# jack-nie/bitcoin-miner

Hardware: AMD Instinct MI355X
Metric: GH/s (SHA-256 nonce search) at 1/2/4/8 MI355X; % of VALU int roofline (higher is better)
Workload: dtype u32

## Files before the change

### bitcoin-miner_amd/csrc/minehip.cpp

```cpp
#include <hip/hip_runtime.h>
#include <stdio.h>
#include <stdlib.h>
#include <string.h>

#include <algorithm>
#include <atomic>
#include <chrono>
#include <cmath>
#include <condition_variable>
#include <memory>
#include <mutex>
#include <string>
#include <system_error>
#include <thread>
#include <vector>

#include "../../include/minehip.h"
#include "../../include/minehip_server.h"
#include "layout.hpp"
#include "msgcodec.hpp"
#include "multi.hpp"
#include "plan.hpp"
#include "sched.hpp"

namespace mh {
hipError_t fast_module_init(int dev);
#ifdef MH_DEV_HOOKS
hipError_t fast_keep_ok(int dev, bool* ok);
#endif
hipError_t launch_fast(int dev, int J, int mode, const FastArgs& a, Partial* partials, hipStream_t s);
hipError_t launch_generic_scan(const GenArgs& a, Partial* partials, uint32_t blocks, hipStream_t s);
hipError_t launch_hash_batch(const GenArgs& a, const uint64_t* d_nonces, uint64_t* d_out, uint64_t n,
                             hipStream_t s);
hipError_t launch_merge(const Partial* partials, uint32_t n, Partial* best, hipStream_t s);
hipError_t launch_batch_scan(const BatchEntry* entries, const uint32_t* tile_entry, Partial* partials, uint32_t tiles,
                             hipStream_t s);
hipError_t launch_merge_segments(const Partial* partials, const uint32_t* seg, Partial* results, uint32_t requests,
                                 hipStream_t s);
}

namespace {

using mh::Partial;

thread_local std::string g_err;

int fail(int code, const std::string& what) {
    g_err = what;
    return code;
}

}

namespace mh {
int set_error(int code, const char* what) { return fail(code, what); }
}

namespace {

#define MH_HIP(call)                                                                                 \
    do {                                                                                             \
        hipError_t e_ = (call);                                                                      \
        if (e_ != hipSuccess) return fail(MH_EHIP, std::string(#call) + ": " + hipGetErrorString(e_)); \
    } while (0)

constexpr uint64_t kBatchChunk = 1u << 22;
constexpr int kEventPairs = 512;
constexpr uint32_t kQueueSlots = 4096;
constexpr size_t kBatchTableBytes = 4u << 20;
constexpr uint32_t kBatchResults = 1u << 16;

struct Timed {
    hipEvent_t start = nullptr, stop = nullptr;
    int kind;
    int var;
};

struct VarStat {
    uint64_t launches = 0, nonces = 0, ns = 0, ops = 0, slots = 0;
};
constexpr int kVariants = 16 * mh::kModes * 5;
inline int var_index(int J, int mode, int L) { return J + 16 * mode + 16 * mh::kModes * (L - 1); }

struct DevCtx {
    std::mutex mu;
    int dev = -1;
    bool ready = false;
    hipStream_t stream = nullptr;
    hipStream_t ps[2] = {nullptr, nullptr};
    hipEvent_t ev_piece[2] = {nullptr, nullptr};
    hipEvent_t ev_main = nullptr;
    Partial* d_partials = nullptr;
    Partial* d_best = nullptr;
    Partial* h_best = nullptr;
    uint64_t* d_nonces = nullptr;
    uint64_t* d_hashes = nullptr;
    uint32_t poff = 0;
    uint32_t* d_counters = nullptr;
    uint32_t qoff = 0;
    uint8_t* d_btab = nullptr;
    uint8_t* h_btab = nullptr;
    Partial* d_bres = nullptr;
    Partial* h_bres = nullptr;
#ifdef MH_DEV_HOOKS
    uint32_t keep = 0;
    bool keep_fast = false;
#endif
    bool prof = false;
    std::vector<Timed> pool;
    int used = 0;
    uint64_t cnt[8] = {0};
    VarStat var[kVariants];
};

std::mutex g_tab_mu;
std::vector<std::unique_ptr<DevCtx>> g_tab;
int g_ndev = -1;

int device_count_impl() {
    std::lock_guard<std::mutex> lk(g_tab_mu);
    if (g_ndev < 0) {
        int n = 0;
        if (hipGetDeviceCount(&n) != hipSuccess) n = 0;
        g_ndev = n;
        g_tab.resize((size_t)n);
        for (auto& p : g_tab) p.reset(new DevCtx());
    }
    return g_ndev;
}

int get_ctx(int dev, DevCtx** out) {
    const int n = device_count_impl();
    if (n <= 0) return fail(MH_ENODEV, "no HIP device visible");
    if (dev < 0 || dev >= n) return fail(MH_EINVAL, "device index out of range");
    DevCtx* c = g_tab[(size_t)dev].get();
    *out = c;
    return MH_OK;
}

int init_locked(DevCtx* c, int dev) {
    if (c->ready) return MH_OK;
    MH_HIP(hipSetDevice(dev));
    hipDeviceProp_t prop;
    MH_HIP(hipGetDeviceProperties(&prop, dev));
    if (strncmp(prop.gcnArchName, "gfx950", 6) != 0)
        return fail(MH_ENODEV, std::string("device is ") + prop.gcnArchName + ", kernels are built for gfx950 only");
    if (!c->stream) MH_HIP(hipStreamCreateWithFlags(&c->stream, hipStreamNonBlocking));
    if (!c->ps[0] || !c->ps[1]) {
        int least = 0, greatest = 0;
        MH_HIP(hipDeviceGetStreamPriorityRange(&least, &greatest));
        if (!c->ps[0]) MH_HIP(hipStreamCreateWithPriority(&c->ps[0], hipStreamNonBlocking, greatest));
        if (!c->ps[1]) MH_HIP(hipStreamCreateWithPriority(&c->ps[1], hipStreamNonBlocking, least));
    }
    for (auto& e : c->ev_piece)
        if (!e) MH_HIP(hipEventCreateWithFlags(&e, hipEventDisableTiming));
    if (!c->ev_main) MH_HIP(hipEventCreateWithFlags(&c->ev_main, hipEventDisableTiming));
    if (!c->d_partials) MH_HIP(hipMalloc(&c->d_partials, sizeof(Partial) * mh::kMaxBlocksPerLaunch));
    if (!c->d_best) MH_HIP(hipMalloc(&c->d_best, sizeof(Partial)));
    if (!c->d_counters) MH_HIP(hipMalloc(&c->d_counters, sizeof(uint32_t) * kQueueSlots));
    if (!c->h_best) MH_HIP(hipHostMalloc(&c->h_best, sizeof(Partial), hipHostMallocDefault));
    if (!c->d_nonces) MH_HIP(hipMalloc(&c->d_nonces, sizeof(uint64_t) * kBatchChunk));
    if (!c->d_hashes) MH_HIP(hipMalloc(&c->d_hashes, sizeof(uint64_t) * kBatchChunk));
    if (c->pool.empty()) c->pool.resize(kEventPairs);
    for (auto& t : c->pool) {
        if (!t.start) MH_HIP(hipEventCreate(&t.start));
        if (!t.stop) MH_HIP(hipEventCreate(&t.stop));
    }
    MH_HIP(mh::fast_module_init(dev));
    c->dev = dev;
    c->ready = true;
    return MH_OK;
}

#ifdef MH_DEV_HOOKS
int read_hash_keep(DevCtx* c) {
    c->keep = 0;
    c->keep_fast = false;
    const char* e = getenv("MINEHIP_DEV_HASH_KEEP");
    if (!e || !*e) return MH_OK;
    unsigned k0 = 0, k1 = 0;
    char rest = 0;
    if (sscanf(e, "%u,%u%c", &k0, &k1, &rest) != 2 || k0 > 32u || k1 > 32u)
        return fail(MH_EINVAL, "MINEHIP_DEV_HASH_KEEP: expected k0,k1 with 0 <= k <= 32");
    MH_HIP(mh::fast_keep_ok(c->dev, &c->keep_fast));
    c->keep = mh::keep_word(k0, k1);
    return MH_OK;
}
#endif

int harvest_locked(DevCtx* c) {
    for (int i = 0; i < c->used; ++i) {
        float ms = 0.f;
        MH_HIP(hipEventElapsedTime(&ms, c->pool[(size_t)i].start, c->pool[(size_t)i].stop));
        const uint64_t ns = (uint64_t)((double)ms * 1.0e6);
        c->cnt[c->pool[(size_t)i].kind == 0 ? 2 : 5] += ns;
        if (c->pool[(size_t)i].kind == 0) c->var[c->pool[(size_t)i].var].ns += ns;
    }
    c->used = 0;
    return MH_OK;
}

int piece_streams_wait_main(DevCtx* c) {
    MH_HIP(hipEventRecord(c->ev_main, c->stream));
    for (auto s : c->ps) MH_HIP(hipStreamWaitEvent(s, c->ev_main, 0));
    return MH_OK;
}

int flush_partials(DevCtx* c, bool split) {
    if (!c->poff) return MH_OK;
    if (split) {
        for (int k = 0; k < 2; ++k) {
            MH_HIP(hipEventRecord(c->ev_piece[k], c->ps[k]));
            MH_HIP(hipStreamWaitEvent(c->stream, c->ev_piece[k], 0));
        }
    }
    MH_HIP(mh::launch_merge(c->d_partials, c->poff, c->d_best, c->stream));
    c->poff = 0;
    if (split) return piece_streams_wait_main(c);
    return MH_OK;
}

bool coarse_piece(const mh::Piece& p, const mh::PlanOpts& opt) { return p.kind == 0 && p.L == opt.lower_digits; }

bool early_piece_ok(const mh::Piece& p) {
    const mh::FastArgs& a = p.fa;
    const uint32_t J = (uint32_t)p.J;
    if ((a.inner >> 2) != J || a.hole + a.hole_w > a.n_hi + a.L) return false;
    for (uint32_t j = 0; j + 1u < a.L; ++j) {
        const uint32_t pos = a.g_last - j - (j >= a.g_hole ? 1u : 0u);
        if (pos > a.g_last || (pos >> 2) != J) return false;
    }
    return true;
}

int enqueue_piece(DevCtx* c, const mh::Piece& p, const mh::PlanOpts& opt, bool split) {
    hipStream_t s = !split ? c->stream : c->ps[coarse_piece(p, opt) ? 0 : 1];
    uint32_t blocks;
    if (p.kind == 0) {
        if (p.fa.n_runs == 0 || p.fa.L < 1 || p.fa.L > 5 || p.fa.n_hi + p.fa.L > 20)
            return fail(MH_EINTERNAL, "internal: bad fast piece");
        if (p.fa.mode >= mh::kModeOneEarly && !early_piece_ok(p))
            return fail(MH_EINTERNAL, "internal: bad Early piece (an enumerated digit outside word J)");
        blocks = (p.fa.n_runs + mh::kBlockThreads - 1) / mh::kBlockThreads;
    } else {
        if (p.ga.count == 0 || p.ga.count > (uint64_t)mh::kMaxBlocksPerLaunch * mh::kBlockThreads)
            return fail(MH_EINTERNAL, "internal: bad generic piece");
        blocks = (uint32_t)((p.ga.count + mh::kBlockThreads - 1) / mh::kBlockThreads);
    }
    if (blocks > mh::kMaxBlocksPerLaunch) return fail(MH_EINTERNAL, "internal: grid too large");
    if (c->poff + blocks > mh::kMaxBlocksPerLaunch) {
        const int rc = flush_partials(c, split);
        if (rc) return rc;
    }
    Partial* out = c->d_partials + c->poff;
    Timed* tm = nullptr;
    mh::FastArgs fa = p.fa;
#ifdef MH_DEV_HOOKS
    mh::GenArgs ga = p.ga;
    ga.pad = c->keep;
    if (p.kind == 0) {
        if (c->keep && !c->keep_fast)
            return fail(MH_EINVAL, "MINEHIP_DEV_HASH_KEEP is set but the fast code object is not the coarse-hash "
                                   "variant (MINEHIP_DEV_CODE_OBJECT=build/fast_search_keep.hsaco)");
        fa.pad_ = c->keep;
    }
#else
    const mh::GenArgs& ga = p.ga;
#endif
    if (p.kind == 0) {
        fa.n_chunks = blocks;
        fa.counter = (opt.queue && c->qoff < kQueueSlots) ? c->d_counters + c->qoff++ : nullptr;
    }
    if (c->prof) {
        if (c->used == kEventPairs) {
            MH_HIP(hipStreamSynchronize(c->stream));
            for (auto ps : c->ps) MH_HIP(hipStreamSynchronize(ps));
            int rc = harvest_locked(c);
            if (rc) return rc;
        }
        tm = &c->pool[(size_t)c->used++];
        tm->kind = p.kind;
        tm->var = p.kind == 0 ? var_index(p.J, p.mode, p.L) : 0;
        MH_HIP(hipEventRecord(tm->start, s));
    }
    if (p.kind == 0)
        MH_HIP(mh::launch_fast(c->dev, p.J, p.mode, fa, out, s));
    else
        MH_HIP(mh::launch_generic_scan(ga, out, blocks, s));
    if (tm) MH_HIP(hipEventRecord(tm->stop, s));
    c->poff += blocks;
    if (c->prof) {
        if (p.kind == 0) {
            const uint64_t n = p.count;
            c->cnt[0] += 1;
            c->cnt[1] += n;
            c->cnt[3] += n * (uint64_t)p.ops;
            c->cnt[6] += n * (uint64_t)p.slots;
            VarStat& v = c->var[var_index(p.J, p.mode, p.L)];
            v.launches += 1;
            v.nonces += n;
            v.ops += n * (uint64_t)p.ops;
            v.slots += n * (uint64_t)p.slots;
        } else {
            c->cnt[4] += p.count;
        }
    }
    return MH_OK;
}

mh::PlanOpts plan_opts() {
    mh::PlanOpts o;
    if (const char* e = getenv("MINEHIP_LOWER_DIGITS")) {
        const int v = atoi(e);
        if (v >= 1 && v <= 5) o.lower_digits = v;
    }
    if (const char* e = getenv("MINEHIP_MIN_LANES")) o.min_lanes = strtoull(e, nullptr, 10);
    if (const char* e = getenv("MINEHIP_LAUNCH_NONCES")) {
        const unsigned long long v = strtoull(e, nullptr, 10);
        if (v >= 1) o.max_nonces_per_launch = v;
    }
    if (const char* e = getenv("MINEHIP_GENERIC_BELOW")) o.generic_below = strtoull(e, nullptr, 10);
    if (const char* e = getenv("MINEHIP_MAX_BLOCKS")) {
        const unsigned long long v = strtoull(e, nullptr, 10);
        if (v >= 1 && v <= mh::kMaxBlocksPerLaunch) o.max_blocks = (uint32_t)v;
    }
    if (const char* e = getenv("MINEHIP_STREAMS")) {
        const int v = atoi(e);
        if (v == 1 || v == 2) o.streams = v;
    }
    if (const char* e = getenv("MINEHIP_FINE_TAIL")) o.fine_tail = strtoull(e, nullptr, 10);
    if (const char* e = getenv("MINEHIP_QUEUE")) {
        const int v = atoi(e);
        if (v == 0 || v == 1) o.queue = v;
    }
    if (const char* e = getenv("MINEHIP_EARLY")) {
        const int v = atoi(e);
        if (v == 0 || v == 1) o.early = v;
    }
    return o;
}

uint64_t now_ns() {
    return (uint64_t)std::chrono::duration_cast<std::chrono::nanoseconds>(
               std::chrono::steady_clock::now().time_since_epoch())
        .count();
}

int search_impl(int dev, const mh::Prefix& pre, uint64_t lower, uint64_t upper, uint64_t* oh, uint64_t* on,
                uint64_t* busy_ns = nullptr) {
    DevCtx* c;
    int rc = get_ctx(dev, &c);
    if (rc) return rc;
    std::lock_guard<std::mutex> lk(c->mu);
    rc = init_locked(c, dev);
    if (rc) return rc;
    const uint64_t t0 = now_ns();
    MH_HIP(hipSetDevice(dev));
#ifdef MH_DEV_HOOKS
    rc = read_hash_keep(c);
    if (rc) return rc;
#endif
    MH_HIP(hipMemsetAsync(c->d_best, 0xFF, sizeof(Partial), c->stream));
    const mh::PlanOpts opt = plan_opts();
    if (opt.queue) MH_HIP(hipMemsetAsync(c->d_counters, 0, sizeof(uint32_t) * kQueueSlots, c->stream));
    c->qoff = 0;
    bool any_coarse = false, any_fine = false;
    if (opt.streams == 2)
        mh::plan_search(pre, lower, upper, opt, [&](const mh::Piece& p) {
            (coarse_piece(p, opt) ? any_coarse : any_fine) = true;
            return !(any_coarse && any_fine);
        });
    const bool split = opt.streams == 2 && any_coarse && any_fine;
    if (split) {
        rc = piece_streams_wait_main(c);
        if (rc) return rc;
    }
    int err = MH_OK;
    c->poff = 0;
    mh::plan_search(pre, lower, upper, opt, [&](const mh::Piece& p) {
        err = enqueue_piece(c, p, opt, split);
        return err == MH_OK;
    });
    if (!err) err = flush_partials(c, split);
    if (err) {
        for (auto ps : c->ps)
            if (ps) (void)hipStreamSynchronize(ps);
        (void)hipStreamSynchronize(c->stream);
        return err;
    }
    MH_HIP(hipMemcpyAsync(c->h_best, c->d_best, sizeof(Partial), hipMemcpyDeviceToHost, c->stream));
    MH_HIP(hipStreamSynchronize(c->stream));
    if (c->prof) {
        rc = harvest_locked(c);
        if (rc) return rc;
    }
    *oh = c->h_best->hash;
    *on = c->h_best->nonce;
    if (busy_ns) *busy_ns = now_ns() - t0;
    return MH_OK;
}

int check_common(const uint8_t* msg, size_t len) {
    if (msg == nullptr && len != 0) return fail(MH_EINVAL, "msg is NULL");
    if (len > MH_MAX_MSG_LEN) return fail(MH_ETOOLONG, "message longer than MH_MAX_MSG_LEN");
    return MH_OK;
}


uint32_t batch_slots() {
    if (const char* e = getenv("MINEHIP_BATCH_SLOTS")) {
        const unsigned long long v = strtoull(e, nullptr, 10);
        if (v >= 1 && v <= mh::kMaxBlocksPerLaunch) return (uint32_t)v;
    }
    return mh::kMaxBlocksPerLaunch;
}

inline size_t align16(size_t x) { return (x + 15u) & ~(size_t)15u; }

int batch_init_locked(DevCtx* c) {
    if (!c->d_btab) MH_HIP(hipMalloc(&c->d_btab, kBatchTableBytes));
    if (!c->h_btab) MH_HIP(hipHostMalloc(&c->h_btab, kBatchTableBytes, hipHostMallocDefault));
    if (!c->d_bres) MH_HIP(hipMalloc(&c->d_bres, sizeof(Partial) * kBatchResults));
    if (!c->h_bres) MH_HIP(hipHostMalloc(&c->h_bres, sizeof(Partial) * kBatchResults, hipHostMallocDefault));
    return MH_OK;
}

struct BatchPending {
    std::vector<size_t> req_idx;
    size_t toff = 0;
};

int batch_drain(DevCtx* c, const mh::BatchRequest* reqs, BatchPending* pend, mh_result* out) {
    MH_HIP(hipStreamSynchronize(c->stream));
    if (c->prof) {
        const int rc = harvest_locked(c);
        if (rc) return rc;
    }
    for (size_t k = 0; k < pend->req_idx.size(); ++k) {
        mh_result& r = out[reqs[pend->req_idx[k]].id];
        r.hash = c->h_bres[k].hash;
        r.nonce = c->h_bres[k].nonce;
    }
    pend->req_idx.clear();
    pend->toff = 0;
    return MH_OK;
}

int batch_run_pass(DevCtx* c, const mh::BatchRequest* reqs, const mh::BatchTables& t, uint32_t slot_cap,
                   BatchPending* pend, mh_result* out) {
    if (!mh::batch_tables_ok(t, slot_cap)) return fail(MH_EINTERNAL, "internal: bad batch tables");
    const size_t ne = t.entries.size(), nreq = t.req_idx.size(), tiles = t.tile_entry.size();
    const size_t o_seg = align16(ne * sizeof(mh::BatchEntry)), o_tile = o_seg + align16((nreq + 1u) * sizeof(uint32_t));
    const size_t bytes = o_tile + align16(tiles * sizeof(uint32_t));
    if (bytes > kBatchTableBytes || nreq > kBatchResults) return fail(MH_EINTERNAL, "internal: batch pass too large");
    if (pend->toff + bytes > kBatchTableBytes || pend->req_idx.size() + nreq > kBatchResults ||
        (c->prof && c->used == kEventPairs)) {
        const int rc = batch_drain(c, reqs, pend, out);
        if (rc) return rc;
    }
    uint8_t* h = c->h_btab + pend->toff;
    uint8_t* d = c->d_btab + pend->toff;
    memcpy(h, t.entries.data(), ne * sizeof(mh::BatchEntry));
#ifdef MH_DEV_HOOKS
    for (size_t i = 0; i < ne; ++i) ((mh::BatchEntry*)h)[i].g.pad = c->keep;
#endif
    memcpy(h + o_seg, t.seg.data(), (nreq + 1u) * sizeof(uint32_t));
    memcpy(h + o_tile, t.tile_entry.data(), tiles * sizeof(uint32_t));
    MH_HIP(hipMemcpyAsync(d, h, bytes, hipMemcpyHostToDevice, c->stream));
    Timed* tm = nullptr;
    if (c->prof) {
        tm = &c->pool[(size_t)c->used++];
        tm->kind = 1;
        tm->var = 0;
// ... 412 lines not shown
```

### bitcoin-miner_amd/csrc/plan.cpp

```cpp
#include "plan.hpp"

#include <string.h>

#include <algorithm>
#include <cmath>

namespace mh {
namespace {

constexpr uint32_t kK[64] = {
    0x428a2f98u, 0x71374491u, 0xb5c0fbcfu, 0xe9b5dba5u, 0x3956c25bu, 0x59f111f1u, 0x923f82a4u, 0xab1c5ed5u,
    0xd807aa98u, 0x12835b01u, 0x243185beu, 0x550c7dc3u, 0x72be5d74u, 0x80deb1feu, 0x9bdc06a7u, 0xc19bf174u,
    0xe49b69c1u, 0xefbe4786u, 0x0fc19dc6u, 0x240ca1ccu, 0x2de92c6fu, 0x4a7484aau, 0x5cb0a9dcu, 0x76f988dau,
    0x983e5152u, 0xa831c66du, 0xb00327c8u, 0xbf597fc7u, 0xc6e00bf3u, 0xd5a79147u, 0x06ca6351u, 0x14292967u,
    0x27b70a85u, 0x2e1b2138u, 0x4d2c6dfcu, 0x53380d13u, 0x650a7354u, 0x766a0abbu, 0x81c2c92eu, 0x92722c85u,
    0xa2bfe8a1u, 0xa81a664bu, 0xc24b8b70u, 0xc76c51a3u, 0xd192e819u, 0xd6990624u, 0xf40e3585u, 0x106aa070u,
    0x19a4c116u, 0x1e376c08u, 0x2748774cu, 0x34b0bcb5u, 0x391c0cb3u, 0x4ed8aa4au, 0x5b9cca4fu, 0x682e6ff3u,
    0x748f82eeu, 0x78a5636fu, 0x84c87814u, 0x8cc70208u, 0x90befffau, 0xa4506cebu, 0xbef9a3f7u, 0xc67178f2u};
constexpr uint32_t kIV[8] = {0x6a09e667u, 0xbb67ae85u, 0x3c6ef372u, 0xa54ff53au,
                             0x510e527fu, 0x9b05688cu, 0x1f83d9abu, 0x5be0cd19u};

inline uint32_t ror(uint32_t x, int n) { return (x >> n) | (x << (32 - n)); }

constexpr uint64_t kPow10[20] = {1ull,
// ... 291 lines not shown
    if (segs.empty() || w.empty()) return;
    using u128 = unsigned __int128;
    double wsum = 0.0;
    for (double x : w) wsum += std::max(0.0, x);
    double total = 0.0;
    for (const CostSeg& s : segs) total += ((double)(s.b - s.a) + 1.0) * s.per;
    const uint64_t lower = segs.front().a;
    const u128 n_all = (u128)(segs.back().b - lower) + 1u;
    u128 prev = 0;
    double acc_w = 0.0;
    for (size_t k = 0; k < w.size(); ++k) {
        acc_w += std::max(0.0, w[k]);
        u128 pos;
        if (k + 1 == w.size() || wsum <= 0.0) {
            pos = (k + 1 == w.size()) ? n_all : prev;
        } else {
            double target = total * (acc_w / wsum), cum = 0.0;
            pos = n_all;
            for (const CostSeg& s : segs) {
                const double len = (double)(s.b - s.a) + 1.0, c = len * s.per;
                if (cum + c >= target) {
                    double n = std::floor((target - cum) / s.per);
                    n = std::min(std::max(n, 0.0), len);
                    pos = (u128)(s.a - lower) + (u128)n;
                    break;
                }
                cum += c;
            }
            if (pos > n_all) pos = n_all;
        }
        if (pos < prev) pos = prev;
        if (pos > prev) (*out)[k] = Span{(uint64_t)(lower + (prev)), (uint64_t)(lower + (pos - 1u)), false};
        prev = pos;
    }
}

void plan_search(const Prefix& pre, uint64_t lower, uint64_t upper, const PlanOpts& opt,
                 const std::function<bool(const Piece&)>& cb) {
    GenArgs gbase;
    make_gen_args(pre, &gbase);
    const int d_lo = decimal_digits(lower), d_hi = decimal_digits(upper);
    const uint64_t max_gen = (uint64_t)std::min(opt.max_blocks, kMaxBlocksPerLaunch) * kBlockThreads;

    bool have_gen = false;
    uint64_t gen_a = 0, gen_b = 0;
    auto flush_generic = [&]() -> bool {
        if (!have_gen) return true;
        have_gen = false;
        Piece p;
        memset(&p, 0, sizeof p);
        p.first = gen_a;
        p.count = gen_b - gen_a + 1u;
        p.kind = 1;
        p.digits = decimal_digits(gen_a);
        p.blocks = ((pre.t + (uint32_t)decimal_digits(gen_b) + 9u) <= 64u) ? 1 : 2;
        p.ga = gbase;
        p.ga.first = gen_a;
        p.ga.count = p.count;
        return cb(p);
    };
    auto emit_generic = [&](uint64_t a, uint64_t b, int) -> bool {
        for (;;) {
            if (have_gen && gen_b - gen_a < max_gen - 1u && gen_b + 1u == a) {
                const uint64_t room = max_gen - 1u - (gen_b - gen_a);
                if (b - a < room) {
                    gen_b = b;
                    return true;
                }
                gen_b = a + (room - 1u);
                a = gen_b + 1u;
            }
            if (!flush_generic()) return false;
            const uint64_t left = b - a;
            const uint64_t cnt = (left >= max_gen - 1u) ? max_gen : left + 1u;
            have_gen = true;
            gen_a = a;
            gen_b = a + (cnt - 1u);
            if (cnt - 1u == left) return true;
            a += cnt;
        }
    };

    auto emit_runs = [&](int d, unsigned __int128 ua, unsigned __int128 ub, uint64_t Bx, int Lx, int Jx, int modex,
                         int nbx, const FastArgs& fax) -> bool {
        const unsigned __int128 Rx = kPow10[Lx];
        const uint64_t lpb = Bx / (uint64_t)Rx;
        uint64_t max_runs = std::min<uint64_t>(max_gen, opt.max_nonces_per_launch / (uint64_t)Rx);
        max_runs = std::max<uint64_t>(lpb, max_runs / lpb * lpb);
        ua *= lpb;
        ub *= lpb;
        for (unsigned __int128 u = ua; u < ub;) {
            const unsigned __int128 left = ub - u;
            const uint64_t runs = (left > max_runs) ? max_runs : (uint64_t)left;
            Piece p;
            memset(&p, 0, sizeof p);
            p.first = (uint64_t)(u * Rx);
            p.count = (uint64_t)((unsigned __int128)runs * Rx);
            p.kind = 0;
            p.digits = d;
            p.L = Lx;
            p.J = Jx;
            p.mode = modex;
            p.blocks = nbx;
            p.fa = fax;
            { const NonceCost nc = nonce_cost(Jx, modex); p.ops = nc.ops; p.slots = nc.slots; }
            p.fa.u_start = (uint64_t)u;
            p.fa.n_runs = (uint32_t)runs;
            p.ga = gbase;
            if (!flush_generic() || !cb(p)) return false;
            u += runs;
        }
        return true;
    };
    auto emit_edge = [&](int d, uint64_t a, uint64_t b) -> bool {
        FastArgs fs;
        int Js = 0, ms = 0, nbs = 1;
        uint64_t bs = 1;
        const int L = 1;
        if (!make_fast_args(pre, d, L, false, &Js, &ms, &nbs, &bs, &fs)) return emit_generic(a, b, d);
        const unsigned __int128 R = bs;
        const unsigned __int128 u0 = ((unsigned __int128)a + R - 1u) / R, u1 = ((unsigned __int128)b + 1u) / R;
        if (u0 >= u1) return emit_generic(a, b, d);
        if (a < (uint64_t)(u0 * R) && !emit_generic(a, (uint64_t)(u0 * R) - 1u, d)) return false;
        if (!emit_runs(d, u0, u1, bs, L, Js, ms, nbs, fs)) return false;
        return u1 * R > (unsigned __int128)b || emit_generic((uint64_t)(u1 * R), b, d);
    };

    for (int d = d_lo; d <= d_hi; ++d) {
        const uint64_t A = std::max(lower, bucket_lo(d)), B = std::min(upper, bucket_hi(d));
        FastArgs fa;
        int L = 0, J = 0, mode = 0, nb = 1;
        uint64_t blk = 1;
        if (!bucket_layout(pre, d, A, B, opt, &L, &J, &mode, &nb, &blk, &fa)) {
            if (!emit_generic(A, B, d)) return;
            continue;
        }
        const bool early = mode >= 3;
        const unsigned __int128 R = blk;
        const unsigned __int128 U0 = ((unsigned __int128)A + R - 1u) / R;
        const unsigned __int128 U1p = ((unsigned __int128)B + 1u) / R;
        if (U0 >= U1p) {
            if (!(early ? emit_edge(d, A, B) : emit_generic(A, B, d))) return;
            continue;
        }
        const uint64_t fast_first = (uint64_t)(U0 * R);
        const unsigned __int128 fast_end = U1p * R;
        if (A < fast_first && !(early ? emit_edge(d, A, fast_first - 1u) : emit_generic(A, fast_first - 1u, d)))
            return;
        unsigned __int128 U_split = U1p;
        int Lf = 0, Jf = 0, modef = 0, nbf = 1;
        uint64_t blkf = 1;
        FastArgs faf;
        if (opt.fine_tail && L == opt.lower_digits && L >= 2) {
            const unsigned __int128 tail_blocks = opt.fine_tail / (uint64_t)R;
            if (tail_blocks >= 1 && (U1p - U0) > 4 * tail_blocks &&
                pick_layout(pre, d, L - 1, A, B, opt, &Jf, &modef, &nbf, &blkf, &faf) && R % blkf == 0u) {
                U_split = U1p - tail_blocks;
                Lf = L - 1;
            }
        }
        if (!emit_runs(d, U0, U_split, blk, L, J, mode, nb, fa)) return;
        if (U_split < U1p && !emit_runs(d, U_split * (R / blkf), U1p * (R / blkf), blkf, Lf, Jf, modef, nbf, faf))
            return;
        if (fast_end <= (unsigned __int128)B &&
            !(early ? emit_edge(d, (uint64_t)fast_end, B) : emit_generic((uint64_t)fast_end, B, d)))
            return;
    }
    flush_generic();
}


uint64_t batch_tiles(uint64_t first, uint64_t count) {
    const uint64_t last = first + (count - 1u);
    const uint64_t decades = last / 10u - first / 10u + 1u;
    return (decades + (kBatchTileDecades - 1u)) / kBatchTileDecades;
}

void plan_batch(const BatchRequest* reqs, size_t n, const PlanOpts& opt, uint32_t slot_cap,
                std::vector<BatchItem>* items) {
    items->clear();
    slot_cap = std::min(slot_cap, kMaxBlocksPerLaunch);
    int pass = 0;
    uint32_t used_slots = 0, used_reqs = 0, used_entries = 0;
    std::vector<BatchItem> mine;
    for (size_t i = 0; i < n; ++i) {
        const BatchRequest& r = reqs[i];
        mine.clear();
        bool fused = true;
        uint64_t tiles = 0;
        plan_search(r.pre, r.lower, r.upper, opt, [&](const Piece& p) {
            if (p.kind != 1 || mine.size() == kBatchMaxEntries) return fused = false;
            const uint64_t t = batch_tiles(p.first, p.count);
            tiles += t;
            if (tiles > slot_cap) return fused = false;
            mine.push_back(BatchItem{r.id, p.first, p.count, 0, 0, 0, (uint32_t)t, i});
            return true;
        });
        if (!fused) {
            items->push_back(BatchItem{r.id, r.lower, r.upper - r.lower + 1u, 1, -1, 0, 0, i});
            continue;
        }
        if (used_reqs && (used_slots + tiles > slot_cap || used_reqs == kBatchMaxRequests ||
                          used_entries + mine.size() > kBatchMaxEntries)) {
            ++pass;
            used_slots = used_reqs = used_entries = 0;
        }
        for (BatchItem& it : mine) {
            it.pass = pass;
            it.slot = used_slots;
            used_slots += it.slots;
            items->push_back(it);
        }
        ++used_reqs;
        used_entries += (uint32_t)mine.size();
    }
}

void build_batch_tables(const BatchRequest* reqs, const std::vector<BatchItem>& items, int pass, BatchTables* out) {
    out->entries.clear();
    out->tile_entry.clear();
    out->seg.clear();
    out->req_idx.clear();
    out->nonces = 0;
    uint32_t slots = 0;
    for (const BatchItem& it : items) {
        if (it.kind != 0 || it.pass != pass) continue;
        if (out->req_idx.empty() || out->req_idx.back() != it.idx) {
            out->req_idx.push_back(it.idx);
            out->seg.push_back(it.slot);
        }
        BatchEntry e;
        make_gen_args(reqs[it.idx].pre, &e.g);
        e.g.first = it.first;
        e.g.count = it.count;
        e.tile0 = it.slot;
        e.slot0 = it.slot;
        out->tile_entry.insert(out->tile_entry.end(), it.slots, (uint32_t)out->entries.size());
        out->entries.push_back(e);
        out->nonces += it.count;
        slots = it.slot + it.slots;
    }
    out->seg.push_back(slots);
}

bool batch_tables_ok(const BatchTables& t, uint32_t slot_cap) {
// ... 28 lines not shown
```

### bitcoin-miner_amd/csrc/plan.hpp

```cpp
#pragma once
#include <stdint.h>
#include <stddef.h>

#include <functional>
#include <vector>

#include "layout.hpp"

namespace mh {

struct Prefix {
    uint32_t mid[8];
    uint8_t tail[64];
    uint32_t t;
    uint64_t plen;
};

void absorb_prefix(const uint8_t* msg, size_t len, Prefix* out);

void host_compress(uint32_t st[8], const uint32_t w16[16]);

struct Piece {
    uint64_t first;
    uint64_t count;
    int kind;
    int digits;
    int L;
    int J;
    int mode;
    int blocks;
    uint32_t ops;
    uint32_t slots;
    FastArgs fa;
    GenArgs ga;
};

struct PlanOpts {
    int lower_digits = 3;
    uint64_t min_lanes = 1u << 19;
    uint64_t max_nonces_per_launch = 1ull << 35;
    uint32_t max_blocks = 1u << 17;
    uint64_t generic_below = 1u << 20;
    int streams = 2;
    uint64_t fine_tail = 1ull << 28;
    int queue = 1;
    int early = 1;
};

void plan_search(const Prefix& pre, uint64_t lower, uint64_t upper, const PlanOpts& opt,
                 const std::function<bool(const Piece&)>& cb);

void make_gen_args(const Prefix& pre, GenArgs* ga);

uint32_t nonce_ops(int J, int mode);

struct NonceCost {
    uint32_t ops, slots;
};
NonceCost nonce_cost(int J, int mode);

int decimal_digits(uint64_t n);

struct CostSeg {
    uint64_t a, b;
    double per;
    bool steady;
};
double unsteady_share(const std::vector<CostSeg>& segs, uint64_t lo, uint64_t hi);
constexpr double kGenericSlotsPerBlock = 2.0 * 1760.0;
constexpr double kUnsteadyFactor = 1.15;
void cost_segments(const Prefix& pre, uint64_t lower, uint64_t upper, const PlanOpts& opt,
                   std::vector<CostSeg>* out);
double segments_cost(const std::vector<CostSeg>& segs, uint64_t lo, uint64_t hi);

struct Span {
    uint64_t lo, hi;
    bool empty;
};
void split_by_cost(const std::vector<CostSeg>& segs, const std::vector<double>& w, std::vector<Span>* out);

struct BatchRequest {
    Prefix pre;
    uint64_t lower, upper;
    uint64_t id;
};

struct BatchItem {
    uint64_t req;
    uint64_t first, count;
    int kind;
    int pass;
    uint32_t slot, slots;
    size_t idx;
};

uint64_t batch_tiles(uint64_t first, uint64_t count);

void plan_batch(const BatchRequest* reqs, size_t n, const PlanOpts& opt, uint32_t slot_cap,
                std::vector<BatchItem>* items);

struct BatchTables {
    std::vector<BatchEntry> entries;
    std::vector<uint32_t> tile_entry;
    std::vector<uint32_t> seg;
    std::vector<size_t> req_idx;
    uint64_t nonces = 0;
};
void build_batch_tables(const BatchRequest* reqs, const std::vector<BatchItem>& items, int pass, BatchTables* out);

bool batch_tables_ok(const BatchTables& t, uint32_t slot_cap);

}
```

### bitcoin-miner_amd/csrc/search_kernels.hip

```cpp
#include <hip/hip_runtime.h>

#include <algorithm>
#include <stdio.h>
#include <stdlib.h>

#include <map>
#include <mutex>
#include <string>
#include <utility>

#include "kernel_common.hpp"
#include "layout.hpp"
#include "sha256_gfx950.hpp"

extern "C" const unsigned char mh_fast_co_begin[];

namespace mh {
namespace dev {

__device__ __forceinline__ void hash_generic(const GenArgs& a, uint64_t n, uint32_t& h0, uint32_t& h1) {
    constexpr uint64_t P10[20] = {1ull, 10ull, 100ull, 1000ull, 10000ull, 100000ull, 1000000ull, 10000000ull,
                                  100000000ull, 1000000000ull, 10000000000ull, 100000000000ull,
                                  1000000000000ull, 10000000000000ull, 100000000000000ull,
                                  1000000000000000ull, 10000000000000000ull, 100000000000000000ull,
                                  1000000000000000000ull, 10000000000000000000ull};
    uint32_t nd = 1;
#pragma unroll
    for (int k = 1; k < 20; ++k) nd += (n >= P10[k]) ? 1u : 0u;
    uint32_t w[32];
#pragma unroll
    for (int x = 0; x < 16; ++x) w[x] = a.tail[x];
#pragma unroll
    for (int x = 16; x < 32; ++x) w[x] = 0u;
    uint64_t u = n;
#pragma unroll
    for (int k = 0; k < 20; ++k) {
        if ((uint32_t)k < nd) {
            const uint64_t q = u / 10u;
            const uint32_t dg = (uint32_t)(u - q * 10u);
            u = q;
            const uint32_t pos = a.t + nd - 1u - (uint32_t)k;
            add_word(w, pos >> 2, (0x30u + dg) << (24u - 8u * (pos & 3u)));
        }
    }
    const uint32_t end = a.t + nd;
    add_word(w, end >> 2, 0x80u << (24u - 8u * (end & 3u)));
    const uint64_t bits = (a.plen + nd) * 8u;
    const bool two = end + 9u > 64u;
    const uint32_t bhi = (uint32_t)(bits >> 32), blo = (uint32_t)bits;
    w[14] = two ? w[14] : bhi;
    w[15] = two ? w[15] : blo;
    w[30] = two ? bhi : 0u;
    w[31] = two ? blo : 0u;
    uint32_t st[8];
#pragma unroll
    for (int i = 0; i < 8; ++i) st[i] = a.mid[i];
    if (!two) {
        sha256_block_h01(st, w, h0, h1);
    } else {
        sha256_block(st, w);
        sha256_block_h01(st, w + 16, h0, h1);
    }
}

}

__global__ __launch_bounds__(kBlockThreads) void generic_scan(const GenArgs a, Partial* __restrict__ partials) {
    using namespace dev;
    const uint32_t gid = blockIdx.x * kBlockThreads + threadIdx.x;
    const uint64_t n = a.first + gid;
    uint32_t h0, h1;
    hash_generic(a, n, h0, h1);
#ifdef MH_DEV_HOOKS
    h0 &= keep_mask0(a.pad);
    h1 &= keep_mask1(a.pad);
#endif
    uint64_t hash = ((uint64_t)h0 << 32) | h1, nonce = n;
    if (gid >= a.count) {
        hash = ~0ull;
        nonce = ~0ull;
    }
    block_min(hash, nonce);
    if (threadIdx.x == 0) partials[blockIdx.x] = Partial{hash, nonce};
}

__global__ __launch_bounds__(kBlockThreads) void hash_batch(const GenArgs a, const uint64_t* __restrict__ nonces,
                                                            uint64_t* __restrict__ out, uint64_t n) {
    const uint64_t i = (uint64_t)blockIdx.x * kBlockThreads + threadIdx.x;
    if (i >= n) return;
    uint32_t h0, h1;
    dev::hash_generic(a, nonces[i], h0, h1);
    out[i] = ((uint64_t)h0 << 32) | h1;
}

constexpr int kMergeThreads = 1024;
constexpr int kMergeUnroll = 8;

__global__ __launch_bounds__(kMergeThreads) void merge_partials(const Partial* __restrict__ p, uint32_t n,
                                                                Partial* __restrict__ best) {
    using namespace dev;
    uint64_t h = ~0ull, nn = ~0ull;
    for (uint32_t base = 0; base < n; base += kMergeThreads * kMergeUnroll) {
        Partial x[kMergeUnroll];
#pragma unroll
        for (int u = 0; u < kMergeUnroll; ++u) {
            const uint32_t i = base + (uint32_t)u * kMergeThreads + threadIdx.x;
            x[u] = (i < n) ? p[i] : Partial{~0ull, ~0ull};
        }
#pragma unroll
        for (int u = 0; u < kMergeUnroll; ++u)
            if (lex_less(x[u].hash, x[u].nonce, h, nn)) {
                h = x[u].hash;
                nn = x[u].nonce;
            }
    }
    block_min<kMergeThreads>(h, nn);
    if (threadIdx.x == 0) {
        const Partial b = *best;
        if (lex_less(h, nn, b.hash, b.nonce)) *best = Partial{h, nn};
    }
}

namespace dev {

__device__ __forceinline__ void scan_decade(const GenArgs& a, uint64_t u, uint32_t jlo, uint32_t jhi, uint64_t& bh,
                                            uint64_t& bn) {
    constexpr uint64_t P10[19] = {1ull, 10ull, 100ull, 1000ull, 10000ull, 100000ull, 1000000ull, 10000000ull,
                                  100000000ull, 1000000000ull, 10000000000ull, 100000000000ull, 1000000000000ull,
                                  10000000000000ull, 100000000000000ull, 1000000000000000ull, 10000000000000000ull,
                                  100000000000000000ull, 1000000000000000000ull};
    uint32_t nu = 0;
#pragma unroll
    for (int k = 0; k < 19; ++k) nu += (u >= P10[k]) ? 1u : 0u;
    uint32_t w[32];
#pragma unroll
    for (int x = 0; x < 16; ++x) w[x] = a.tail[x];
#pragma unroll
    for (int x = 16; x < 32; ++x) w[x] = 0u;
    uint64_t q = u;
#pragma unroll
    for (int k = 0; k < 19; ++k) {
        if ((uint32_t)k < nu) {
            const uint64_t q10 = q / 10u;
            const uint32_t dg = (uint32_t)(q - q10 * 10u);
            q = q10;
            const uint32_t pos = a.t + nu - 1u - (uint32_t)k;
            add_word(w, pos >> 2, (0x30u + dg) << (24u - 8u * (pos & 3u)));
        }
    }
    const uint32_t last = a.t + nu;
    const uint32_t lsh = 24u - 8u * (last & 3u);
    add_word(w, last >> 2, 0x30u << lsh);
    const uint32_t end = last + 1u;
    add_word(w, end >> 2, 0x80u << (24u - 8u * (end & 3u)));
    const uint64_t bits = (a.plen + nu + 1u) * 8u;
    const bool two = end + 9u > 64u;
    const uint32_t bhi = (uint32_t)(bits >> 32), blo = (uint32_t)bits;
    w[14] = two ? w[14] : bhi;
    w[15] = two ? w[15] : blo;
    w[30] = two ? bhi : 0u;
    w[31] = two ? blo : 0u;
    const bool in1 = last >= 64u;
    const bool both = two && !in1;
    const uint32_t jw = (last >> 2) & 15u;
    uint32_t st[8];
#pragma unroll
    for (int i = 0; i < 8; ++i) st[i] = a.mid[i];
    if (in1) sha256_block(st, w);
    uint32_t v[16];
#pragma unroll
    for (int x = 0; x < 16; ++x) {
        const uint32_t lo = w[x], hi = w[16 + x];
        v[x] = in1 ? hi : lo;
    }
    const uint32_t w16 = w[16];
    const uint64_t n0 = u * 10u;
#pragma unroll 1
    for (uint32_t j = jlo; j <= jhi; ++j) {
        const uint32_t dj = j << lsh;
        uint32_t x[16];
#pragma unroll
        for (int i = 0; i < 16; ++i) x[i] = v[i] | ((jw == (uint32_t)i) ? dj : 0u);
        uint32_t s[8];
#pragma unroll
        for (int i = 0; i < 8; ++i) s[i] = st[i];
        if (both) {
            sha256_block(s, x);
#pragma unroll
            for (int i = 0; i < 16; ++i) x[i] = 0u;
            x[0] = w16;
            x[14] = bhi;
            x[15] = blo;
        }
        uint32_t h0, h1;
        sha256_block_h01(s, x, h0, h1);
#ifdef MH_DEV_HOOKS
        h0 &= keep_mask0(a.pad);
        h1 &= keep_mask1(a.pad);
#endif
        const uint64_t hash = ((uint64_t)h0 << 32) | h1, n = n0 + j;
        if (lex_less(hash, n, bh, bn)) {
            bh = hash;
            bn = n;
// ... 114 lines not shown
#ifdef MH_DEV_HOOKS
hipError_t fast_keep_ok(int dev, bool* ok) {
    hipFunction_t f;
    *ok = false;
    const hipError_t e = fast_function(dev, 4, kModeOne, &f);
    if (e != hipSuccess) return e;
    const char* co = getenv("MINEHIP_DEV_CODE_OBJECT");
    std::lock_guard<std::mutex> g(g_mod_mu);
    const auto it = g_mods.find({(co && *co) ? co : "", dev});
    if (it != g_mods.end()) *ok = g_keep_ok[it->second];
    return hipSuccess;
}
#endif

hipError_t resident_groups(int dev, hipFunction_t f, unsigned lds, uint32_t* out) {
    static std::mutex mu;
    static std::map<std::pair<hipFunction_t, unsigned>, uint32_t> cache;
    std::lock_guard<std::mutex> g(mu);
    auto it = cache.find({f, lds});
    if (it == cache.end()) {
        int per_cu = 0, cus = 0;
        hipError_t e = hipModuleOccupancyMaxActiveBlocksPerMultiprocessor(&per_cu, f, kBlockThreads, lds);
        if (e == hipSuccess) e = hipDeviceGetAttribute(&cus, hipDeviceAttributeMultiprocessorCount, dev);
        if (e != hipSuccess) {
            (void)hipGetLastError();
            return e;
        }
        it = cache.emplace(std::make_pair(f, lds), (uint32_t)std::max(1, per_cu) * (uint32_t)std::max(1, cus)).first;
    }
    *out = it->second;
    return hipSuccess;
}

hipError_t launch_fast(int dev, int J, int mode, const FastArgs& a, Partial* partials, hipStream_t s) {
    if (!fast_variant_exists(J, mode)) return hipErrorInvalidValue;
#ifdef MH_DEV_HOOKS
    const char* lds_env = getenv("MINEHIP_DEV_LDS");
    const unsigned lds = lds_env ? (unsigned)atoi(lds_env) : 0u;
#else
    constexpr unsigned lds = 0;
#endif
    hipFunction_t f;
    bool queue_ok = false;
    hipError_t e = fast_function(dev, J, mode, &f, &queue_ok);
    if (e != hipSuccess) return e;
    FastArgs args = a;
    if (!queue_ok) args.counter = nullptr;
    uint32_t grid = args.n_chunks;
    if (args.counter) {
        uint32_t resident = 0;
        e = resident_groups(dev, f, lds, &resident);
        if (e != hipSuccess) return e;
        grid = std::min(grid, resident);
    }
    Partial* out = partials;
    void* params[] = {&args, &out};
    return hipModuleLaunchKernel(f, grid, 1, 1, kBlockThreads, 1, 1, lds, s, params, nullptr);
}

hipError_t launch_generic_scan(const GenArgs& a, Partial* partials, uint32_t blocks, hipStream_t s) {
    hipLaunchKernelGGL(generic_scan, dim3(blocks), dim3(kBlockThreads), 0, s, a, partials);
    return hipGetLastError();
}

hipError_t launch_hash_batch(const GenArgs& a, const uint64_t* d_nonces, uint64_t* d_out, uint64_t n,
                             hipStream_t s) {
    const uint64_t blocks = (n + kBlockThreads - 1) / kBlockThreads;
    hipLaunchKernelGGL(hash_batch, dim3((uint32_t)blocks), dim3(kBlockThreads), 0, s, a, d_nonces, d_out, n);
    return hipGetLastError();
}

hipError_t launch_batch_scan(const BatchEntry* entries, const uint32_t* tile_entry, Partial* partials, uint32_t tiles,
                             hipStream_t s) {
    hipLaunchKernelGGL(batch_scan, dim3(tiles), dim3(kBlockThreads), 0, s, entries, tile_entry, partials);
    return hipGetLastError();
}

hipError_t launch_merge_segments(const Partial* partials, const uint32_t* seg, Partial* results, uint32_t requests,
                                 hipStream_t s) {
    hipLaunchKernelGGL(merge_segments, dim3(requests), dim3(kBlockThreads), 0, s, partials, seg, results);
    return hipGetLastError();
}

hipError_t launch_merge(const Partial* partials, uint32_t n, Partial* best, hipStream_t s) {
    hipLaunchKernelGGL(merge_partials, dim3(1), dim3(kMergeThreads), 0, s, partials, n, best);
    return hipGetLastError();
}

}
```

Before: 52.22.

## Gate fine-stream tail pieces on coarse stream progress via event

Adds a StreamPlan that records an event on the coarse stream before each coarse launch and makes tail fine pieces wait on that event before launching on the fine stream. This delays tail fine work until the preceding coarse work has started, so the low-priority fine stream does not compete for CUs too early and the tail overlaps better with coarse work. The gate is on by default and can be turned off with MINEHIP_TAIL_GATE. It adds extra event record and wait calls and may serialize the streams more than needed.

```diff
diff --git a/bitcoin-miner_amd/csrc/minehip.cpp b/bitcoin-miner_amd/csrc/minehip.cpp
--- a/bitcoin-miner_amd/csrc/minehip.cpp
+++ b/bitcoin-miner_amd/csrc/minehip.cpp
@@ -21,6 +21,7 @@
 #include "msgcodec.hpp"
 #include "multi.hpp"
 #include "plan.hpp"
+#include "stream_plan.hpp"
 #include "sched.hpp"
 
 namespace mh {
@@ -90,6 +91,7 @@
     hipStream_t ps[2] = {nullptr, nullptr};
     hipEvent_t ev_piece[2] = {nullptr, nullptr};
     hipEvent_t ev_main = nullptr;
+    hipEvent_t ev_gate = nullptr;
     Partial* d_partials = nullptr;
     Partial* d_best = nullptr;
     Partial* h_best = nullptr;
@@ -155,6 +157,7 @@
     for (auto& e : c->ev_piece)
         if (!e) MH_HIP(hipEventCreateWithFlags(&e, hipEventDisableTiming));
     if (!c->ev_main) MH_HIP(hipEventCreateWithFlags(&c->ev_main, hipEventDisableTiming));
+    if (!c->ev_gate) MH_HIP(hipEventCreateWithFlags(&c->ev_gate, hipEventDisableTiming));
     if (!c->d_partials) MH_HIP(hipMalloc(&c->d_partials, sizeof(Partial) * mh::kMaxBlocksPerLaunch));
     if (!c->d_best) MH_HIP(hipMalloc(&c->d_best, sizeof(Partial)));
     if (!c->d_counters) MH_HIP(hipMalloc(&c->d_counters, sizeof(uint32_t) * kQueueSlots));
@@ -220,8 +223,6 @@
     return MH_OK;
 }
 
-bool coarse_piece(const mh::Piece& p, const mh::PlanOpts& opt) { return p.kind == 0 && p.L == opt.lower_digits; }
-
 bool early_piece_ok(const mh::Piece& p) {
     const mh::FastArgs& a = p.fa;
     const uint32_t J = (uint32_t)p.J;
@@ -233,8 +234,10 @@
     return true;
 }
 
-int enqueue_piece(DevCtx* c, const mh::Piece& p, const mh::PlanOpts& opt, bool split) {
-    hipStream_t s = !split ? c->stream : c->ps[coarse_piece(p, opt) ? 0 : 1];
+int enqueue_piece(DevCtx* c, const mh::Piece& p, const mh::PlanOpts& opt, bool split, mh::StreamPlan* sp) {
+    const mh::PieceOps ops = sp->next(p);
+    auto stream_of = [&](int k) { return k == mh::kStreamMain ? c->stream : c->ps[k]; };
+    hipStream_t s = stream_of(ops.stream());
     uint32_t blocks;
     if (p.kind == 0) {
         if (p.fa.n_runs == 0 || p.fa.L < 1 || p.fa.L > 5 || p.fa.n_hi + p.fa.L > 20)
@@ -270,6 +273,12 @@
     if (p.kind == 0) {
         fa.n_chunks = blocks;
         fa.counter = (opt.queue && c->qoff < kQueueSlots) ? c->d_counters + c->qoff++ : nullptr;
+    }
+    for (int i = 0; i + 1 < ops.n; ++i) {
+        if (ops.op[i].kind == mh::kOpRecord)
+            MH_HIP(hipEventRecord(c->ev_gate, stream_of(ops.op[i].stream)));
+        else
+            MH_HIP(hipStreamWaitEvent(stream_of(ops.op[i].stream), c->ev_gate, 0));
     }
     if (c->prof) {
         if (c->used == kEventPairs) {
@@ -337,6 +346,10 @@
         const int v = atoi(e);
         if (v == 0 || v == 1) o.early = v;
     }
+    if (const char* e = getenv("MINEHIP_TAIL_GATE")) {
+        const int v = atoi(e);
+        if (v == 0 || v == 1) o.tail_gate = v;
+    }
     return o;
 }
 
@@ -367,7 +380,7 @@
     bool any_coarse = false, any_fine = false;
     if (opt.streams == 2)
         mh::plan_search(pre, lower, upper, opt, [&](const mh::Piece& p) {
-            (coarse_piece(p, opt) ? any_coarse : any_fine) = true;
+            (mh::coarse_piece(p, opt) ? any_coarse : any_fine) = true;
             return !(any_coarse && any_fine);
         });
     const bool split = opt.streams == 2 && any_coarse && any_fine;
@@ -377,8 +390,9 @@
     }
     int err = MH_OK;
     c->poff = 0;
+    mh::StreamPlan sp(opt, split);
     mh::plan_search(pre, lower, upper, opt, [&](const mh::Piece& p) {
-        err = enqueue_piece(c, p, opt, split);
+        err = enqueue_piece(c, p, opt, split, &sp);
         return err == MH_OK;
     });
     if (!err) err = flush_partials(c, split);
diff --git a/bitcoin-miner_amd/csrc/plan.cpp b/bitcoin-miner_amd/csrc/plan.cpp
--- a/bitcoin-miner_amd/csrc/plan.cpp
+++ b/bitcoin-miner_amd/csrc/plan.cpp
@@ -397,7 +397,7 @@
     };
 
     auto emit_runs = [&](int d, unsigned __int128 ua, unsigned __int128 ub, uint64_t Bx, int Lx, int Jx, int modex,
-                         int nbx, const FastArgs& fax) -> bool {
+                         int nbx, const FastArgs& fax, bool tail = false) -> bool {
         const unsigned __int128 Rx = kPow10[Lx];
         const uint64_t lpb = Bx / (uint64_t)Rx;
         uint64_t max_runs = std::min<uint64_t>(max_gen, opt.max_nonces_per_launch / (uint64_t)Rx);
@@ -422,6 +422,7 @@
             p.fa.u_start = (uint64_t)u;
             p.fa.n_runs = (uint32_t)runs;
             p.ga = gbase;
+            p.tail = tail;
             if (!flush_generic() || !cb(p)) return false;
             u += runs;
         }
@@ -475,7 +476,8 @@
             }
         }
         if (!emit_runs(d, U0, U_split, blk, L, J, mode, nb, fa)) return;
-        if (U_split < U1p && !emit_runs(d, U_split * (R / blkf), U1p * (R / blkf), blkf, Lf, Jf, modef, nbf, faf))
+        if (U_split < U1p &&
+            !emit_runs(d, U_split * (R / blkf), U1p * (R / blkf), blkf, Lf, Jf, modef, nbf, faf, true))
             return;
         if (fast_end <= (unsigned __int128)B &&
             !(early ? emit_edge(d, (uint64_t)fast_end, B) : emit_generic((uint64_t)fast_end, B, d)))
diff --git a/bitcoin-miner_amd/csrc/plan.hpp b/bitcoin-miner_amd/csrc/plan.hpp
--- a/bitcoin-miner_amd/csrc/plan.hpp
+++ b/bitcoin-miner_amd/csrc/plan.hpp
@@ -33,6 +33,7 @@
     uint32_t slots;
     FastArgs fa;
     GenArgs ga;
+    bool tail;
 };
 
 struct PlanOpts {
@@ -45,6 +46,7 @@
     uint64_t fine_tail = 1ull << 28;
     int queue = 1;
     int early = 1;
+    int tail_gate = 1;
 };
 
 void plan_search(const Prefix& pre, uint64_t lower, uint64_t upper, const PlanOpts& opt,
diff --git a/bitcoin-miner_amd/csrc/stream_plan.hpp b/bitcoin-miner_amd/csrc/stream_plan.hpp
--- /dev/null
+++ b/bitcoin-miner_amd/csrc/stream_plan.hpp
@@ -0,0 +1,58 @@
+#pragma once
+#include "plan.hpp"
+
+namespace mh {
+
+constexpr int kStreamMain = -1;
+constexpr int kStreamCoarse = 0;
+constexpr int kStreamFine = 1;
+
+enum StreamOpKind {
+    kOpRecord = 0,
+    kOpWait = 1,
+    kOpLaunch = 2,
+};
+
+struct StreamOp {
+    int kind;
+    int stream;
+};
+
+struct PieceOps {
+    StreamOp op[2];
+    int n;
+    int stream() const { return op[n - 1].stream; }
+};
+
+inline bool coarse_piece(const Piece& p, const PlanOpts& opt) { return p.kind == 0 && p.L == opt.lower_digits; }
+
+class StreamPlan {
+  public:
+    StreamPlan(const PlanOpts& opt, bool split) : opt_(opt), split_(split), gate_(split && opt.tail_gate != 0) {}
+
+    PieceOps next(const Piece& p) {
+        PieceOps o{};
+        if (!split_) {
+            o.op[o.n++] = StreamOp{kOpLaunch, kStreamMain};
+            return o;
+        }
+        if (coarse_piece(p, opt_)) {
+            if (gate_) {
+                o.op[o.n++] = StreamOp{kOpRecord, kStreamCoarse};
+                recorded_ = true;
+            }
+            o.op[o.n++] = StreamOp{kOpLaunch, kStreamCoarse};
+            return o;
+        }
+        if (gate_ && p.tail && recorded_) o.op[o.n++] = StreamOp{kOpWait, kStreamFine};
+        o.op[o.n++] = StreamOp{kOpLaunch, kStreamFine};
+        return o;
+    }
+
+  private:
+    PlanOpts opt_;
+    bool split_, gate_;
+    bool recorded_ = false;
+};
+
+}
```

Result: no change. 52.34 (median of 6 runs) (+0.2%).

## Fold best-reset, counter clear and result copy into final merge kernel

Applied to the files above, without the earlier changes.

Drops the per-search memsets of the best record and queue counters and the device-to-host copy. The final merge kernel now seeds from scratch on its first call, writes the result directly into coherent pinned host memory, and zeroes the used counters itself. Generic pieces are also steered onto the low-priority piece stream when no fine fast pieces exist, and the initial cross-stream wait is removed. This cuts per-call launches and host work for short searches, but relies on counters staying zeroed across calls and on correct cross-stream ordering without the initial event wait.

```diff
diff --git a/bitcoin-miner_amd/csrc/minehip.cpp b/bitcoin-miner_amd/csrc/minehip.cpp
--- a/bitcoin-miner_amd/csrc/minehip.cpp
+++ b/bitcoin-miner_amd/csrc/minehip.cpp
@@ -32,7 +32,8 @@
 hipError_t launch_generic_scan(const GenArgs& a, Partial* partials, uint32_t blocks, hipStream_t s);
 hipError_t launch_hash_batch(const GenArgs& a, const uint64_t* d_nonces, uint64_t* d_out, uint64_t n,
                              hipStream_t s);
-hipError_t launch_merge(const Partial* partials, uint32_t n, Partial* best, hipStream_t s);
+hipError_t launch_merge(const Partial* partials, uint32_t n, Partial* best, bool first, Partial* result,
+                        uint32_t* counters, uint32_t n_counters, hipStream_t s);
 hipError_t launch_batch_scan(const BatchEntry* entries, const uint32_t* tile_entry, Partial* partials, uint32_t tiles,
                              hipStream_t s);
 hipError_t launch_merge_segments(const Partial* partials, const uint32_t* seg, Partial* results, uint32_t requests,
@@ -93,6 +94,9 @@
     Partial* d_partials = nullptr;
     Partial* d_best = nullptr;
     Partial* h_best = nullptr;
+    Partial* d_hbest = nullptr;
+    bool merged = false;
+    bool low_fast = false;
     uint64_t* d_nonces = nullptr;
     uint64_t* d_hashes = nullptr;
     uint32_t poff = 0;
@@ -157,8 +161,18 @@
     if (!c->ev_main) MH_HIP(hipEventCreateWithFlags(&c->ev_main, hipEventDisableTiming));
     if (!c->d_partials) MH_HIP(hipMalloc(&c->d_partials, sizeof(Partial) * mh::kMaxBlocksPerLaunch));
     if (!c->d_best) MH_HIP(hipMalloc(&c->d_best, sizeof(Partial)));
-    if (!c->d_counters) MH_HIP(hipMalloc(&c->d_counters, sizeof(uint32_t) * kQueueSlots));
-    if (!c->h_best) MH_HIP(hipHostMalloc(&c->h_best, sizeof(Partial), hipHostMallocDefault));
+    if (!c->d_counters) {
+        uint32_t* p = nullptr;
+        MH_HIP(hipMalloc(&p, sizeof(uint32_t) * kQueueSlots));
+        const hipError_t e = hipMemset(p, 0, sizeof(uint32_t) * kQueueSlots);
+        if (e != hipSuccess) {
+            (void)hipFree(p);
+            return fail(MH_EHIP, std::string("hipMemset(counters): ") + hipGetErrorString(e));
+        }
+        c->d_counters = p;
+    }
+    if (!c->h_best) MH_HIP(hipHostMalloc(&c->h_best, sizeof(Partial), hipHostMallocCoherent));
+    if (!c->d_hbest) MH_HIP(hipHostGetDevicePointer((void**)&c->d_hbest, c->h_best, 0));
     if (!c->d_nonces) MH_HIP(hipMalloc(&c->d_nonces, sizeof(uint64_t) * kBatchChunk));
     if (!c->d_hashes) MH_HIP(hipMalloc(&c->d_hashes, sizeof(uint64_t) * kBatchChunk));
     if (c->pool.empty()) c->pool.resize(kEventPairs);
@@ -206,18 +220,31 @@
     return MH_OK;
 }
 
-int flush_partials(DevCtx* c, bool split) {
-    if (!c->poff) return MH_OK;
+int flush_partials(DevCtx* c, bool split, bool last) {
+    if (!c->poff && !last) return MH_OK;
     if (split) {
         for (int k = 0; k < 2; ++k) {
             MH_HIP(hipEventRecord(c->ev_piece[k], c->ps[k]));
             MH_HIP(hipStreamWaitEvent(c->stream, c->ev_piece[k], 0));
         }
     }
-    MH_HIP(mh::launch_merge(c->d_partials, c->poff, c->d_best, c->stream));
+    MH_HIP(mh::launch_merge(c->d_partials, c->poff, c->d_best, !c->merged, last ? c->d_hbest : nullptr,
+                            last ? c->d_counters : nullptr, last ? c->qoff : 0u, c->stream));
+    c->merged = true;
     c->poff = 0;
-    if (split) return piece_streams_wait_main(c);
-    return MH_OK;
+    if (last) c->qoff = 0;
+    if (split && !last) return piece_streams_wait_main(c);
+    return MH_OK;
+}
+
+void reset_counters(DevCtx* c) {
+    for (auto ps : c->ps)
+        if (ps) (void)hipStreamSynchronize(ps);
+    (void)hipStreamSynchronize(c->stream);
+    (void)hipMemsetAsync(c->d_counters, 0, sizeof(uint32_t) * kQueueSlots, c->stream);
+    (void)hipStreamSynchronize(c->stream);
+    (void)hipGetLastError();
+    c->qoff = 0;
 }
 
 bool coarse_piece(const mh::Piece& p, const mh::PlanOpts& opt) { return p.kind == 0 && p.L == opt.lower_digits; }
@@ -234,7 +261,13 @@
 }
 
 int enqueue_piece(DevCtx* c, const mh::Piece& p, const mh::PlanOpts& opt, bool split) {
-    hipStream_t s = !split ? c->stream : c->ps[coarse_piece(p, opt) ? 0 : 1];
+    hipStream_t s = c->stream;
+    if (split && p.kind == 0) {
+        s = c->ps[coarse_piece(p, opt) ? 0 : 1];
+        if (s == c->ps[1]) c->low_fast = true;
+    } else if (split && !c->low_fast) {
+        s = c->ps[1];
+    }
     uint32_t blocks;
     if (p.kind == 0) {
         if (p.fa.n_runs == 0 || p.fa.L < 1 || p.fa.L > 5 || p.fa.n_hi + p.fa.L > 20)
@@ -249,7 +282,7 @@
     }
     if (blocks > mh::kMaxBlocksPerLaunch) return fail(MH_EINTERNAL, "internal: grid too large");
     if (c->poff + blocks > mh::kMaxBlocksPerLaunch) {
-        const int rc = flush_partials(c, split);
+        const int rc = flush_partials(c, split, false);
         if (rc) return rc;
     }
     Partial* out = c->d_partials + c->poff;
@@ -360,10 +393,10 @@
     rc = read_hash_keep(c);
     if (rc) return rc;
 #endif
-    MH_HIP(hipMemsetAsync(c->d_best, 0xFF, sizeof(Partial), c->stream));
     const mh::PlanOpts opt = plan_opts();
-    if (opt.queue) MH_HIP(hipMemsetAsync(c->d_counters, 0, sizeof(uint32_t) * kQueueSlots, c->stream));
     c->qoff = 0;
+    c->merged = false;
+    c->low_fast = false;
     bool any_coarse = false, any_fine = false;
     if (opt.streams == 2)
         mh::plan_search(pre, lower, upper, opt, [&](const mh::Piece& p) {
@@ -371,24 +404,17 @@
             return !(any_coarse && any_fine);
         });
     const bool split = opt.streams == 2 && any_coarse && any_fine;
-    if (split) {
-        rc = piece_streams_wait_main(c);
-        if (rc) return rc;
-    }
     int err = MH_OK;
     c->poff = 0;
     mh::plan_search(pre, lower, upper, opt, [&](const mh::Piece& p) {
         err = enqueue_piece(c, p, opt, split);
         return err == MH_OK;
     });
-    if (!err) err = flush_partials(c, split);
+    if (!err) err = flush_partials(c, split, true);
     if (err) {
-        for (auto ps : c->ps)
-            if (ps) (void)hipStreamSynchronize(ps);
-        (void)hipStreamSynchronize(c->stream);
+        reset_counters(c);
         return err;
     }
-    MH_HIP(hipMemcpyAsync(c->h_best, c->d_best, sizeof(Partial), hipMemcpyDeviceToHost, c->stream));
     MH_HIP(hipStreamSynchronize(c->stream));
     if (c->prof) {
         rc = harvest_locked(c);
diff --git a/bitcoin-miner_amd/csrc/search_kernels.hip b/bitcoin-miner_amd/csrc/search_kernels.hip
--- a/bitcoin-miner_amd/csrc/search_kernels.hip
+++ b/bitcoin-miner_amd/csrc/search_kernels.hip
@@ -97,7 +97,10 @@
 constexpr int kMergeUnroll = 8;
 
 __global__ __launch_bounds__(kMergeThreads) void merge_partials(const Partial* __restrict__ p, uint32_t n,
-                                                                Partial* __restrict__ best) {
+                                                                Partial* __restrict__ best, uint32_t first,
+                                                                Partial* __restrict__ result,
+                                                                uint32_t* __restrict__ counters,
+                                                                uint32_t n_counters) {
     using namespace dev;
     uint64_t h = ~0ull, nn = ~0ull;
     for (uint32_t base = 0; base < n; base += kMergeThreads * kMergeUnroll) {
@@ -116,9 +119,21 @@
     }
     block_min<kMergeThreads>(h, nn);
     if (threadIdx.x == 0) {
-        const Partial b = *best;
-        if (lex_less(h, nn, b.hash, b.nonce)) *best = Partial{h, nn};
-    }
+        if (!first) {
+            const Partial b = *best;
+            if (!lex_less(h, nn, b.hash, b.nonce)) {
+                h = b.hash;
+                nn = b.nonce;
+            }
+        }
+        if (result) {
+            *result = Partial{h, nn};
+            __threadfence_system();
+        } else {
+            *best = Partial{h, nn};
+        }
+    }
+    for (uint32_t i = threadIdx.x; i < n_counters; i += kMergeThreads) counters[i] = 0u;
 }
 
 namespace dev {
@@ -399,8 +414,10 @@
     return hipGetLastError();
 }
 
-hipError_t launch_merge(const Partial* partials, uint32_t n, Partial* best, hipStream_t s) {
-    hipLaunchKernelGGL(merge_partials, dim3(1), dim3(kMergeThreads), 0, s, partials, n, best);
+hipError_t launch_merge(const Partial* partials, uint32_t n, Partial* best, bool first, Partial* result,
+                        uint32_t* counters, uint32_t n_counters, hipStream_t s) {
+    hipLaunchKernelGGL(merge_partials, dim3(1), dim3(kMergeThreads), 0, s, partials, n, best, first ? 1u : 0u, result,
+                       counters, n_counters);
     return hipGetLastError();
 }
 
```

Result: no change. 54.70 before, 54.76 after (median of 3 runs) (+0.1%).
